# better62/MM-VQA-Healthcare

Hardware: AMD Instinct MI355X
Metric: image-question pairs/sec, M3AE-base fine-tune step (fwd+bwd+AdamW) @384px (higher is better)
Workload: dtype bf16

## Files before the change

### include/m3ae_hip.h

```cpp
#ifndef M3AE_HIP_H
#define M3AE_HIP_H

#include <stdint.h>

#ifdef __cplusplus
extern "C" {
#endif

#define M3AE_ABI_VERSION 4

enum { M3AE_F32 = 0, M3AE_BF16 = 1 };
enum { M3AE_ACT_NONE = 0, M3AE_ACT_GELU = 1, M3AE_ACT_QUICKGELU = 2, M3AE_ACT_TANH = 3, M3AE_ACT_RELU = 4,
       M3AE_ACT_MULAUX = 5  };
enum { M3AE_ERR_ARG = -1, M3AE_ERR_UNSUPPORTED = -2, M3AE_ERR_ALIGN = -3, M3AE_ERR_WORKSPACE = -4 };

int m3ae_abi_version(void);
void m3ae_desc_sizes(int64_t out3[3]);
const char* m3ae_last_gemm_path(void);

typedef struct {
    int64_t M, N, K;
    int64_t batch1, batch2;
    const void* A; int64_t a_sm, a_sk, a_sb1, a_sb2;
    const void* B; int64_t b_sk, b_sn, b_sb1, b_sb2;
    void* C;       int64_t c_sm, c_sn, c_sb1, c_sb2;
    int32_t dtype_a, dtype_b, dtype_c;
    float alpha;
    int32_t accumulate;
    const float* bias;
    int32_t act;
    void* preact;
    const void* residual;
    const void* dact_aux;
    int32_t dact;
    int32_t force_generic;
    float* a_rowsum;
    float dropout_p;
    uint64_t dropout_seed;
    int32_t preact_grad;
    int32_t launch_flags;
    const void* dropout_salt;
} m3ae_gemm_desc;
enum { M3AE_GEMM_NO_PERSISTENT = 1,
       M3AE_GEMM_F32_X3 = 2,
       M3AE_GEMM_DETERMINISTIC = 4,
       M3AE_GEMM_B_TILED = 8    };
#define M3AE_GEMM_NT_VARIANT(v) ((((v) + 1) & 0xf) << 8)
#define M3AE_GEMM_TN_VARIANT(v) ((((v) + 1) & 0xf) << 12)
#define M3AE_GEMM_COL_GROUP(g) (((g) & 0xf) << 16)
int m3ae_gemm(const m3ae_gemm_desc* d, void* stream);
int m3ae_gemm_rows(const m3ae_gemm_desc* d, int64_t row_base, int64_t row_step, void* stream);
int64_t m3ae_gemm_det_workspace_bytes(const m3ae_gemm_desc* d);
int m3ae_gemm_det(const m3ae_gemm_desc* d, void* workspace, int64_t workspace_bytes, void* stream);

typedef struct {
    int64_t B, H, Lq, Lk, Dh;
    const void* q; int64_t q_sb, q_sl;
    const void* k; int64_t k_sb, k_sl;
    const void* v; int64_t v_sb, v_sl;
    void* o;       int64_t o_sb, o_sl;
    const float* key_mask;
    const float* pos_bias;
    float scale;
    int32_t causal;
    float* lse; int64_t lse_stride;
    int32_t dtype;
    void* workspace; int64_t workspace_bytes;
    const void* d_o;
    void* dq; void* dk; void* dv;
    float* delta;
    float* d_pos_bias;
    float dropout_p;
    uint64_t dropout_seed;
    const void* dropout_salt;
    int32_t launch_flags;
} m3ae_attn_desc;
enum { M3AE_ATTN_LEGACY_KERNELS = 1,
       M3AE_ATTN_F32_X3 = 2    };
int64_t m3ae_attn_workspace_bytes(const m3ae_attn_desc* d, int backward);
int m3ae_attn_fwd(const m3ae_attn_desc* d, void* stream);
int m3ae_attn_bwd(const m3ae_attn_desc* d, void* stream);
int m3ae_attn_fwd_rows(const m3ae_attn_desc* d, int64_t row_base, int64_t row_step, void* stream);
int m3ae_attn_bwd_rows(const m3ae_attn_desc* d, int64_t row_base, int64_t row_step, void* stream);
int m3ae_attn_probs(const m3ae_attn_desc* d, float* probs, int64_t p_sb, int64_t p_sh, int64_t p_sq, void* stream);

typedef struct {
    int32_t dir;
    int64_t B, Lq, Lk, D, H;
    const void* x;
    const void* y;
    const float* key_mask;
    const void *wq, *wq_t, *wkv, *wkv_t, *wo, *wo_t;
    const float *bq, *bkv, *bo, *ln_g, *ln_b;
    float ln_eps;
    float dropout_p;
    uint64_t seed_attn, seed_hidden;
    void* proj;
    void* prime;
    float* colbias;
    void* probs;
    void* probs_drop;
    float* rowsum;
    void* zctx;
    void* ctx;
    void* s;
    void* out;
    float *mean, *rstd;
    const void* d_out;
    void* dx;
    void* dy;
    float *g_wq, *g_wkv, *g_wo, *g_bq, *g_bkv, *g_bo, *g_ln_g, *g_ln_b;
    void* ws_ds;
    void* ws_dsd;
    void* ws_dscores;
    void* ws_dprime;
    void* ws_dproj;
    void* ws_dz;
    void* ws_dctx;
    float* ws_vec;
    float* ws_ln;
    int32_t launch_flags;
    const void* dropout_salt;
} m3ae_xattn_desc;
enum { M3AE_XATTN_NO_PERSISTENT = 1,
       M3AE_XATTN_LEGACY_CHAIN = 2     };
int m3ae_xattn_supported(const m3ae_xattn_desc* d);
int m3ae_xattn_bwd_supported(const m3ae_xattn_desc* d);
int64_t m3ae_xattn_probs_ld(const m3ae_xattn_desc* d);
int m3ae_xattn_fwd(const m3ae_xattn_desc* d, void* stream);
int m3ae_xattn_bwd(const m3ae_xattn_desc* d, void* stream);
int m3ae_xattn_probs_export(const m3ae_xattn_desc* d, int dropped, float* out, int64_t o_sb, int64_t o_sh, int64_t o_sq,
                            void* stream);

int m3ae_layernorm_fwd(const void* x, const float* gamma, const float* beta, void* y, float* mean, float* rstd,
// ... 135 lines not shown
```

### mm-vqa-healthcare_amd/csrc/gemm_mfma.hip

```cpp
#include "gemm_nt_common.h"
#include "launch.h"
#include <stdlib.h>

namespace {

constexpr int BM = 128, BN = 128, BK = 64;
constexpr int STAGE_BYTES = (BM + BN) * BK * 2;
constexpr int LDS_BYTES = 2 * STAGE_BYTES;

using namespace m3g;

template <int BM_, int BN_, int BKT, int NST, int WM, int EPI>
__global__ __launch_bounds__((BM_ / WM) * (BN_ / 64) * 64, 2) void gemm_nt_bf16_kernel(MfmaArgs a) {
    if (a.has_drop) drop_resolve(a.drop);
    constexpr int WAVES_N = BN_ / 64, NWAVES = (BM_ / WM) * WAVES_N, MI = WM / 16;
    constexpr int A_BYTES = BM_ * BKT * 2, ST_BYTES = (BM_ + BN_) * BKT * 2;
    constexpr int A_SEGS = A_BYTES / 1024 / NWAVES, B_SEGS = BN_ * BKT * 2 / 1024 / NWAVES;
    constexpr int G = A_SEGS + B_SEGS;
    extern __shared__ __attribute__((aligned(16))) char smem[];
    const int tid = threadIdx.x;
    const int lane = tid & 63;
    const int wave = __builtin_amdgcn_readfirstlane(tid >> 6);
    const int wr = wave / WAVES_N, wc = wave % WAVES_N;

// ... 282 lines not shown
            for (int j = 0; j < 4; ++j)
                acc[i][j] = __builtin_amdgcn_mfma_f32_16x16x32_bf16(
                    __builtin_bit_cast(bf16x8_t, bfr[j]), __builtin_bit_cast(bf16x8_t, af[i]), acc[i][j], 0, 0, 0);
        __builtin_amdgcn_s_setprio(0);
        PP_FENCE();
        __builtin_amdgcn_s_barrier();
        PP_FENCE();
#pragma unroll
        for (int i = 0; i < 4; ++i) af[i] = nt_frag<CK>(At, wr * 128 + 64 + i * 16 + frow, fchunk);
        if (more) nt_stage<CK, 2, NW>(a.A, a.lda, m0, a.M, (int64_t)(c + 3) * CK, nxt, wave, lane);
        {
            const int rem = nc - 1 - c;
            if (rem >= 3) asm volatile("s_waitcnt vmcnt(8)" ::: "memory");
            else if (rem == 2) asm volatile("s_waitcnt vmcnt(4)" ::: "memory");
            else asm volatile("s_waitcnt vmcnt(0)" ::: "memory");
        }
        PP_FENCE();
        __builtin_amdgcn_s_barrier();
        PP_FENCE();
        asm volatile("s_waitcnt lgkmcnt(0)" ::: "memory");
        __builtin_amdgcn_sched_barrier(0);
        __builtin_amdgcn_s_setprio(1);
#pragma unroll
        for (int i = 0; i < 4; ++i)
#pragma unroll
            for (int j = 0; j < 4; ++j)
                acc[4 + i][j] = __builtin_amdgcn_mfma_f32_16x16x32_bf16(
                    __builtin_bit_cast(bf16x8_t, bfr[j]), __builtin_bit_cast(bf16x8_t, af[i]), acc[4 + i][j], 0, 0, 0);
        __builtin_amdgcn_s_setprio(0);
        PP_FENCE();
        __builtin_amdgcn_s_barrier();
        PP_FENCE();
    }
    if (wr == 0) { __builtin_amdgcn_s_barrier(); PP_FENCE(); }

    if (a.rows_epi) {
        if (a.c_f32) epilogue_rows<float, EPI, 8>(a, smem, wave, lane, m0 + wr * 128, n0 + wc * 64, acc);
        else epilogue_rows<bf16_t, EPI, 8>(a, smem, wave, lane, m0 + wr * 128, n0 + wc * 64, acc);
        return;
    }
#pragma unroll
    for (int i = 0; i < 8; ++i) {
        const int64_t m = m0 + wr * 128 + i * 16 + (lane & 15);
        if (m >= a.M) continue;
#pragma unroll
        for (int j = 0; j < 4; ++j) {
            const int64_t n = n0 + wc * 64 + j * 16 + 4 * (lane >> 4);
            if (n >= a.N) continue;
            if (a.c_f32) epilogue4<float, EPI>(a, m, n, acc[i][j]);
            else epilogue4<bf16_t, EPI>(a, m, n, acc[i][j]);
        }
    }
}

template <int EPI>
static int launch_nt_pp(const MfmaArgs& a, hipStream_t s) {
    constexpr int lds = 4 * (256 + 256) * 32 * 2;
    const int64_t tiles = cdiv(a.M, 256) * cdiv(a.N, 256);
    return launch_dyn<gemm_nt_pp_kernel<EPI>>(dim3((unsigned)tiles), dim3(512), lds, s, a);
}

enum NtKernel { NT_T128, NT_T256, NT_PP, NT_PP2, NT_PP2_PERSISTENT };

static NtKernel nt_kernel_choice(const MfmaArgs& a) {
    const bool both = a.M > 128 && a.N > 128;
    const bool pp2_ok = both && a.rows_epi && a.K >= 256;
    if (a.nt_variant >= 0) {
        switch (a.nt_variant) {
        case 9: return pp2_ok ? NT_PP2 : NT_T128;
        case 10: return pp2_ok ? NT_PP2_PERSISTENT : NT_T128;
        case 7: return both ? NT_PP : NT_T128;
        case 4: return both ? NT_T256 : NT_T128;
        default: return NT_T128;
        }
    }
    const int64_t t256 = cdiv(a.M, 256) * cdiv(a.N, 256), t128 = cdiv(a.M, 128) * cdiv(a.N, 128);
    const double eff256 = (double)t256 / (double)(cdiv(t256, 256) * 256);
    const double eff128 = (double)t128 / (double)(cdiv(t128, 512) * 512);
    if (!both || eff256 < 0.93 * eff128) return NT_T128;
    if (!pp2_ok) return NT_PP;
    return t256 >= 512 && !a.no_persist ? NT_PP2_PERSISTENT : NT_PP2;
}

template <int EPI>
static int launch_nt_v(const MfmaArgs& a, hipStream_t s) {
    const NtKernel k = nt_kernel_choice(a);
    g_last_path = k == NT_PP ? "mfma_nt_pp" : (k == NT_PP2 || k == NT_PP2_PERSISTENT) ? "mfma_nt_pp2" : "mfma_nt";
    switch (k) {
    case NT_PP2: return launch_nt_pp2(a, EPI, false, s);
    case NT_PP2_PERSISTENT: return launch_nt_pp2(a, EPI, true, s);
    case NT_PP: return launch_nt_pp<EPI>(a, s);
    case NT_T256: return launch_nt_t<256, 256, 64, 2, 128, EPI>(a, s);
    default: return launch_nt_t<128, 128, 64, 2, 64, EPI>(a, s);
    }
}


static int launch_nt(const m3ae_gemm_desc& d, hipStream_t s, DropRows rows) {
    MfmaArgs a{};
    a.A = (const bf16_t*)d.A; a.lda = d.a_sm;
    a.B = (const bf16_t*)d.B; a.ldb = d.b_sn;
    a.C = d.C; a.ldc = d.c_sm;
    a.M = d.M; a.N = d.N; a.K = d.K;
    a.c_f32 = d.dtype_c == M3AE_F32;
    a.alpha = d.alpha; a.accumulate = d.accumulate; a.bias = d.bias; a.act = d.act; a.preact = d.preact;
    a.preact_grad = d.preact_grad;
    a.residual = d.residual; a.dact_aux = d.dact_aux; a.dact = d.dact;
    a.rows_epi = (d.N % 8 == 0 && d.c_sm % 8 == 0) ? 1 : 0;
    {
        const int tiles_n = (int)((d.N + 255) / 256);
        const int g_nt_col_group = (d.launch_flags >> 16) & 0xf;
        a.col_group = g_nt_col_group > 0 ? g_nt_col_group : (tiles_n <= 9 ? tiles_n : 6);
    }
    a.has_drop = d.dropout_p > 0.f;
    a.drop = make_drop(d.dropout_p, d.dropout_seed, d.dropout_salt, rows);
    a.no_persist = (d.launch_flags & M3AE_GEMM_NO_PERSISTENT) ? 1 : 0;
    a.nt_variant = ((d.launch_flags >> 8) & 0xf) - 1;
    a.b_tiled = (d.launch_flags & M3AE_GEMM_B_TILED) ? 1 : 0;
    a.st_policy = (d.launch_flags >> 20) & 0x3;
    if (a.st_policy == 0) a.st_policy = (d.M * d.N >= (int64_t)16 << 20) ? 3 : 1;
    const bool has_act = d.act != M3AE_ACT_NONE, has_dact = d.dact_aux != nullptr;
    if (!has_act && !has_dact && !d.preact) return launch_nt_v<EPI_PLAIN>(a, s);
    if (!has_dact && d.act == M3AE_ACT_RELU) return launch_nt_v<EPI_RELU>(a, s);
    if (!has_act && has_dact && d.dact == M3AE_ACT_MULAUX) return launch_nt_v<EPI_DMUL>(a, s);
    if (a.has_drop) return launch_nt_v<EPI_ANY>(a, s);
    if (!has_dact && d.act == M3AE_ACT_GELU) return launch_nt_v<EPI_GELU>(a, s);
    if (!has_dact && d.act == M3AE_ACT_QUICKGELU) return launch_nt_v<EPI_QGELU>(a, s);
    if (!has_act && d.dact == M3AE_ACT_GELU) return launch_nt_v<EPI_DGELU>(a, s);
    if (!has_act && d.dact == M3AE_ACT_QUICKGELU) return launch_nt_v<EPI_DQGELU>(a, s);
    return launch_nt_v<EPI_ANY>(a, s);
}


#ifdef M3AE_TN_TRACE
__device__ uint64_t g_tn_trace[512 * 2 * 16];
#define TN_STAMP(k) do { if (tn_tr) g_tn_trace[((size_t)blockIdx.x * 2 + wr) * 16 + (k)] = __builtin_readcyclecounter(); } while (0)
extern "C" int m3ae_tn_trace_dump(uint64_t* out) {
    hipDeviceSynchronize();
    hipMemcpyFromSymbol(out, HIP_SYMBOL(g_tn_trace), sizeof(uint64_t) * 512 * 2 * 16);
    static uint64_t zeros[512 * 2 * 16];
    hipMemcpyToSymbol(HIP_SYMBOL(g_tn_trace), zeros, sizeof(zeros));
    return 0;
}
#else
#define TN_STAMP(k) do { } while (0)
#endif
template <bool DET>
__global__ __launch_bounds__(512, 2) void gemm_tn_pp_kernel(MfmaArgs a) {
    constexpr int CK = 32, NW = 8, A_BYTES = 256 * CK * 2, SLOT = 2 * A_BYTES;
    extern __shared__ __attribute__((aligned(16))) char smem[];
    const int tid = threadIdx.x;
    const int lane = tid & 63;
    const int wave = __builtin_amdgcn_readfirstlane(tid >> 6);
    const int wr = wave >> 2, wc = wave & 3;

    const unsigned tiles_n = (unsigned)(a.N / 256);
    const unsigned tiles = (unsigned)(a.M / 256) * tiles_n;
    const unsigned wg = xcd_remap(blockIdx.x, gridDim.x);
    const unsigned tile_id = wg % tiles, split = wg / tiles;
    const int64_t m0 = (int64_t)(tile_id / tiles_n) * 256;
    const int64_t n0 = (int64_t)(tile_id % tiles_n) * 256;
    const int64_t r_begin = (int64_t)split * a.k_chunk;
    int64_t r_end = r_begin + a.k_chunk;
    if (r_end > a.K) r_end = a.K;
    if (r_begin >= r_end) return;
    const int nc = (int)((r_end - r_begin + CK - 1) / CK);

    f32x4 acc[8][4];
#pragma unroll
    for (int i = 0; i < 8; ++i)
#pragma unroll
        for (int j = 0; j < 4; ++j) acc[i][j] = (f32x4){0.f, 0.f, 0.f, 0.f};
    const bool do_rowsum = a.a_rowsum != nullptr && n0 == 0 && wc == 0;
    f32x4 rsum[8];
#pragma unroll
    for (int i = 0; i < 8; ++i) rsum[i] = (f32x4){0.f, 0.f, 0.f, 0.f};
    const s16x8 ones = {0x3F80, 0x3F80, 0x3F80, 0x3F80, 0x3F80, 0x3F80, 0x3F80, 0x3F80};

#pragma unroll
    for (int c = 0; c < 3; ++c) {
        if (c < nc) {
            const int64_t r0 = r_begin + (int64_t)c * CK;
            tn_stage<256, 2, NW>(a.B, a.ldb, r0, r_end, n0, smem + c * SLOT + A_BYTES, wave, lane);
            tn_stage<256, 2, NW>(a.A, a.lda, r0, r_end, m0, smem + c * SLOT, wave, lane);
        }
    }
    if (nc >= 3) asm volatile("s_waitcnt vmcnt(8)" ::: "memory");
    else if (nc == 2) asm volatile("s_waitcnt vmcnt(4)" ::: "memory");
    else asm volatile("s_waitcnt vmcnt(0)" ::: "memory");
    PP_FENCE();
    __builtin_amdgcn_s_barrier();
    PP_FENCE();
    if (wr == 1) { __builtin_amdgcn_s_barrier(); PP_FENCE(); }

    for (int c = 0; c < nc; ++c) {
#ifdef M3AE_TN_TRACE
        const bool tn_tr = (c == 64 || c == 65) && lane == 0 && wc == 0 && blockIdx.x < 512;
        if (tn_tr && c == 65) g_tn_trace[((size_t)blockIdx.x * 2 + wr) * 16 + 8] = __builtin_readcyclecounter();
#undef TN_STAMP
#define TN_STAMP(k) do { if (tn_tr && c == 64) g_tn_trace[((size_t)blockIdx.x * 2 + wr) * 16 + (k)] = __builtin_readcyclecounter(); } while (0)
#endif
        TN_STAMP(0);
        const char* At = smem + (c & 3) * SLOT;
        const char* Bt = At + A_BYTES;
        char* nxt = smem + ((c + 3) & 3) * SLOT;
        const bool more = c + 3 < nc;
        const int64_t r3 = r_begin + (int64_t)(c + 3) * CK;
        s16x8 bfr[4], af[4];
#pragma unroll
        for (int j = 0; j < 4; ++j) bfr[j] = tn_frag<256>(Bt, 0, wc * 64 + j * 16, lane);
#pragma unroll
        for (int i = 0; i < 4; ++i) af[i] = tn_frag<256>(At, 0, wr * 128 + i * 16, lane);
        if (more) tn_stage<256, 2, NW>(a.B, a.ldb, r3, r_end, n0, nxt + A_BYTES, wave, lane);
// ... 212 lines not shown
}

static int tn_kernel_choice(const m3ae_gemm_desc& d) {
    const bool pp_ok = d.M % 256 == 0 && d.N % 256 == 0 && d.K >= 4096;
    const int g_tn_variant = ((d.launch_flags >> 12) & 0xf) - 1;
    if (g_tn_variant == 5 && pp_ok) return 5;
    if (g_tn_variant < 0 || g_tn_variant == 6) {
        const bool r3_rule = pp_ok && (d.K >= 65536 || (d.K >= 32768 && d.M * d.N >= 768 * 3072));
        const bool r4_rule = pp_ok && d.K >= 65536 && d.M * d.N >= 768 * 3072;
        if (g_tn_variant == 6 ? r3_rule : r4_rule) return 5;
        return 2;
    }
    if (g_tn_variant == 2) return 2;
    return 0;
}

static int launch_tn(const m3ae_gemm_desc& d, hipStream_t s, float* det_ws = nullptr) {
    MfmaArgs a{};
    a.A = (const bf16_t*)d.A; a.lda = d.a_sk;
    a.B = (const bf16_t*)d.B; a.ldb = d.b_sk;
    a.C = d.C; a.ldc = d.c_sm;
    a.M = d.M; a.N = d.N; a.K = d.K;
    a.c_f32 = 1; a.alpha = d.alpha; a.accumulate = d.accumulate; a.a_rowsum = d.a_rowsum;
    const int k = tn_kernel_choice(d);
    if (k == 5) return launch_tn_pp(a, d, s, det_ws);
    if (k == 2) return launch_tn_t<128, 128, 64, 32, 2>(a, d, s, det_ws);
    return launch_tn_t<128, 128, 64, 64, 2>(a, d, s, det_ws);
}


enum GemmRoute { ROUTE_BAD_DIMS, ROUTE_F32X3, ROUTE_NT, ROUTE_TN, ROUTE_GENERIC };
static GemmRoute gemm_route(const m3ae_gemm_desc& d) {
    if (d.M <= 0 || d.N <= 0 || d.K <= 0 || d.batch1 <= 0 || d.batch2 <= 0) return ROUTE_BAD_DIMS;
    if ((d.launch_flags & M3AE_GEMM_F32_X3) && !d.force_generic) return ROUTE_F32X3;
    const bool bf = d.dtype_a == M3AE_BF16 && d.dtype_b == M3AE_BF16;
    const bool single = d.batch1 == 1 && d.batch2 == 1;
    if (bf && single && !d.force_generic && d.c_sn == 1) {
        const bool ptr_ok = aligned16(d.A) && aligned16(d.B) && aligned16(d.C) &&
                            (!d.preact || aligned16(d.preact)) && (!d.residual || aligned16(d.residual)) &&
                            (!d.dact_aux || aligned16(d.dact_aux)) && (!d.bias || aligned16(d.bias));
        if (ptr_ok && !d.a_rowsum && d.a_sk == 1 && d.b_sk == 1 && d.K % BK == 0 && d.N % 4 == 0 && d.a_sm % 8 == 0 &&
            d.b_sn % 8 == 0 && d.c_sm % 4 == 0)
            return ROUTE_NT;
        if (ptr_ok && d.a_sm == 1 && d.b_sn == 1 && d.dtype_c == M3AE_F32 && d.M % BM == 0 && d.N % BN == 0 &&
            d.a_sk % 8 == 0 && d.b_sk % 8 == 0 && !d.bias && d.act == M3AE_ACT_NONE && !d.preact && !d.residual &&
            !d.dact_aux)
            return ROUTE_TN;
    }
    return ROUTE_GENERIC;
}

extern "C" int m3ae_gemm(const m3ae_gemm_desc* dp, void* stream) { return m3ae_gemm_rows(dp, 0, 1, stream); }

extern "C" int m3ae_gemm_rows(const m3ae_gemm_desc* dp, int64_t row_base, int64_t row_step, void* stream) {
    if (!dp || !dp->A || !dp->B || !dp->C) return M3AE_ERR_ARG;
    const m3ae_gemm_desc& d = *dp;
    const GemmRoute route = gemm_route(d);
    if (route == ROUTE_BAD_DIMS) return M3AE_ERR_ARG;
    const DropRows rows{row_base, row_step};
    if (!drop_rows_ok(rows, d.M, d.N)) return M3AE_ERR_ARG;
    if ((d.launch_flags & M3AE_GEMM_B_TILED) &&
        (d.dtype_a != M3AE_BF16 || d.dtype_b != M3AE_BF16 || d.b_sk != 1 || d.b_sn != d.K || d.K % 32 != 0 || d.batch1 != 1 ||
         d.batch2 != 1 || (d.launch_flags & M3AE_GEMM_F32_X3) || !aligned16(d.B)))
        return M3AE_ERR_UNSUPPORTED;
    if (route == ROUTE_TN && d.dropout_p > 0.f && (row_base != 0 || row_step != 1)) return M3AE_ERR_UNSUPPORTED;
    if (d.launch_flags & M3AE_GEMM_DETERMINISTIC) return M3AE_ERR_UNSUPPORTED;
    hipStream_t s = (hipStream_t)stream;
    switch (route) {
    case ROUTE_F32X3:
        if (d.dtype_a != M3AE_F32 || d.dtype_b != M3AE_F32 || d.dtype_c != M3AE_F32) return M3AE_ERR_UNSUPPORTED;
        g_last_path = "f32x3";
        return m3ae_gemm_f32x3(d, s, rows);
    case ROUTE_NT:
        return launch_nt(d, s, rows);
    case ROUTE_TN:
        g_last_path = "mfma_tn";
        return launch_tn(d, s);
    default:
        g_last_path = "generic";
        return m3ae_gemm_generic(d, s, rows);
    }
}

extern "C" int64_t m3ae_gemm_det_workspace_bytes(const m3ae_gemm_desc* dp) {
    if (!dp) return M3AE_ERR_ARG;
    const m3ae_gemm_desc& d = *dp;
    if (gemm_route(d) != ROUTE_TN) return 0;
    int64_t k_chunk = 0;
    const int k = tn_kernel_choice(d);
    const int64_t splits = k == 5 ? tn_pp_splits(d, &k_chunk) : tn_t_splits(d, tn_t_lds(2, k == 2 ? 32 : 64), &k_chunk);
    return tn_det_bytes(d, splits);
}

extern "C" int m3ae_gemm_det(const m3ae_gemm_desc* dp, void* workspace, int64_t workspace_bytes, void* stream) {
    if (!dp || !dp->A || !dp->B || !dp->C) return M3AE_ERR_ARG;
    const m3ae_gemm_desc& d = *dp;
    if (!(d.launch_flags & M3AE_GEMM_DETERMINISTIC)) return M3AE_ERR_ARG;
    if (d.launch_flags & M3AE_GEMM_B_TILED) return M3AE_ERR_UNSUPPORTED;
    if (gemm_route(d) != ROUTE_TN) return M3AE_ERR_UNSUPPORTED;
    if (!workspace || !aligned16(workspace) || workspace_bytes < m3ae_gemm_det_workspace_bytes(dp)) return M3AE_ERR_WORKSPACE;
    g_last_path = "mfma_tn";
    return launch_tn(d, (hipStream_t)stream, (float*)workspace);
}
```

### mm-vqa-healthcare_amd/m3ae_amd/_lib.py

```python
import ctypes as C
import os

_PKG = os.path.dirname(os.path.abspath(__file__))
DIAGNOSTIC = os.environ.get("M3AE_DIAGNOSTIC_LIB", "") == "1"
LIB_PATH = os.path.join(_PKG, "lib_diag" if DIAGNOSTIC else "lib", "libm3ae_hip.so")

F32, BF16 = 0, 1
ACT_NONE, ACT_GELU, ACT_QUICKGELU, ACT_TANH, ACT_RELU, ACT_MULAUX = 0, 1, 2, 3, 4, 5

vp, i64, i32, f32 = C.c_void_p, C.c_int64, C.c_int32, C.c_float


class GemmDesc(C.Structure):
    _fields_ = [
        ("M", i64), ("N", i64), ("K", i64), ("batch1", i64), ("batch2", i64),
        ("A", vp), ("a_sm", i64), ("a_sk", i64), ("a_sb1", i64), ("a_sb2", i64),
        ("B", vp), ("b_sk", i64), ("b_sn", i64), ("b_sb1", i64), ("b_sb2", i64),
        ("C", vp), ("c_sm", i64), ("c_sn", i64), ("c_sb1", i64), ("c_sb2", i64),
        ("dtype_a", i32), ("dtype_b", i32), ("dtype_c", i32),
        ("alpha", f32), ("accumulate", i32), ("bias", vp), ("act", i32), ("preact", vp), ("residual", vp),
        ("dact_aux", vp), ("dact", i32), ("force_generic", i32), ("a_rowsum", vp),
        ("dropout_p", f32), ("dropout_seed", C.c_uint64), ("preact_grad", i32), ("launch_flags", i32), ("dropout_salt", vp),
    ]


class AttnDesc(C.Structure):
    _fields_ = [
        ("B", i64), ("H", i64), ("Lq", i64), ("Lk", i64), ("Dh", i64),
        ("q", vp), ("q_sb", i64), ("q_sl", i64),
        ("k", vp), ("k_sb", i64), ("k_sl", i64),
        ("v", vp), ("v_sb", i64), ("v_sl", i64),
        ("o", vp), ("o_sb", i64), ("o_sl", i64),
        ("key_mask", vp), ("pos_bias", vp), ("scale", f32), ("causal", i32),
        ("lse", vp), ("lse_stride", i64), ("dtype", i32), ("workspace", vp), ("workspace_bytes", i64),
        ("d_o", vp), ("dq", vp), ("dk", vp), ("dv", vp), ("delta", vp), ("d_pos_bias", vp),
        ("dropout_p", f32), ("dropout_seed", C.c_uint64), ("dropout_salt", vp), ("launch_flags", i32),
    ]


class XattnDesc(C.Structure):
    _fields_ = [
        ("dir", i32), ("B", i64), ("Lq", i64), ("Lk", i64), ("D", i64), ("H", i64),
        ("x", vp), ("y", vp), ("key_mask", vp),
        ("wq", vp), ("wq_t", vp), ("wkv", vp), ("wkv_t", vp), ("wo", vp), ("wo_t", vp),
        ("bq", vp), ("bkv", vp), ("bo", vp), ("ln_g", vp), ("ln_b", vp),
        ("ln_eps", f32), ("dropout_p", f32), ("seed_attn", C.c_uint64), ("seed_hidden", C.c_uint64),
        ("proj", vp), ("prime", vp), ("colbias", vp), ("probs", vp), ("probs_drop", vp), ("rowsum", vp),
        ("zctx", vp), ("ctx", vp), ("s", vp), ("out", vp), ("mean", vp), ("rstd", vp),
        ("d_out", vp), ("dx", vp), ("dy", vp),
        ("g_wq", vp), ("g_wkv", vp), ("g_wo", vp), ("g_bq", vp), ("g_bkv", vp), ("g_bo", vp), ("g_ln_g", vp), ("g_ln_b", vp),
        ("ws_ds", vp), ("ws_dsd", vp), ("ws_dscores", vp), ("ws_dprime", vp), ("ws_dproj", vp), ("ws_dz", vp), ("ws_dctx", vp),
        ("ws_vec", vp), ("ws_ln", vp), ("launch_flags", i32), ("dropout_salt", vp),
    ]


GEMM_NO_PERSISTENT, GEMM_F32_X3, GEMM_DETERMINISTIC, GEMM_B_TILED = 1, 2, 4, 8
DET_COLSUM, DET_EMBED_BWD, DET_BCE, DET_XENT, DET_MIM = 0, 1, 2, 3, 4
ATTN_LEGACY_KERNELS, ATTN_F32_X3 = 1, 2
XATTN_NO_PERSISTENT, XATTN_LEGACY_CHAIN = 1, 2
CLIP_NORM, CLIP_COEF, CLIP_SKIP, CLIP_STEPS, CLIP_CLIPPED_STEPS, CLIP_SKIPPED_STEPS, CLIP_RECORD_WORDS = 0, 1, 2, 4, 5, 6, 8
ABI_VERSION = 4


_SIGS = {
    "m3ae_abi_version": (C.c_int, []),
    "m3ae_desc_sizes": (None, [C.POINTER(i64)]),
    "m3ae_last_gemm_path": (C.c_char_p, []),
    "m3ae_gemm": (C.c_int, [C.POINTER(GemmDesc), vp]),
    "m3ae_attn_workspace_bytes": (i64, [C.POINTER(AttnDesc), C.c_int]),
    "m3ae_attn_fwd": (C.c_int, [C.POINTER(AttnDesc), vp]),
    "m3ae_attn_bwd": (C.c_int, [C.POINTER(AttnDesc), vp]),
    "m3ae_attn_probs": (C.c_int, [C.POINTER(AttnDesc), vp, i64, i64, i64, vp]),
    "m3ae_xattn_supported": (C.c_int, [C.POINTER(XattnDesc)]),
    "m3ae_xattn_bwd_supported": (C.c_int, [C.POINTER(XattnDesc)]),
    "m3ae_xattn_probs_ld": (i64, [C.POINTER(XattnDesc)]),
    "m3ae_xattn_fwd": (C.c_int, [C.POINTER(XattnDesc), vp]),
    "m3ae_xattn_bwd": (C.c_int, [C.POINTER(XattnDesc), vp]),
    "m3ae_xattn_probs_export": (C.c_int, [C.POINTER(XattnDesc), C.c_int, vp, i64, i64, i64, vp]),
    "m3ae_layernorm_fwd": (C.c_int, [vp, vp, vp, vp, vp, vp, i64, i64, f32, C.c_int, C.c_int, C.c_int, vp]),
    "m3ae_layernorm_bwd_blocks": (i64, [i64]),
    "m3ae_layernorm_bwd": (C.c_int, [vp, vp, vp, vp, vp, vp, vp, vp, vp, vp, vp, i64, i64, C.c_int, C.c_int, C.c_int, vp]),
    "m3ae_layernorm_bwd_drop": (C.c_int, [vp, vp, vp, vp, vp, vp, vp, vp, f32, C.c_uint64, vp, vp, vp, vp, i64, i64, C.c_int, vp]),
    "m3ae_dropout": (C.c_int, [vp, vp, vp, i64, i64, f32, C.c_uint64, vp, C.c_int, vp]),
    "m3ae_colsum": (C.c_int, [vp, vp, i64, i64, i64, C.c_int, C.c_int, vp]),
    "m3ae_roberta_embed_fwd": (C.c_int, [vp, vp, vp, vp, vp, i64, i64, i64, i64, C.c_int, vp]),
    "m3ae_roberta_embed_bwd": (C.c_int, [vp, vp, vp, vp, vp, i64, i64, i64, i64, C.c_int, vp]),
    "m3ae_patchify": (C.c_int, [vp, vp, i64, i64, i64, C.c_int, vp]),
    "m3ae_image_normalize_u8": (C.c_int, [vp, vp, i64, i64, i64, C.POINTER(C.c_float), C.POINTER(C.c_float), vp]),
    "m3ae_vit_tokens_fwd": (C.c_int, [vp, vp, vp, vp, i64, i64, i64, C.c_int, vp]),
    "m3ae_vit_tokens_bwd": (C.c_int, [vp, vp, vp, vp, i64, i64, i64, C.c_int, vp]),
    "m3ae_bce_logits": (C.c_int, [vp, vp, vp, vp, i64, i64, f32, C.c_int, vp]),
    "m3ae_xent": (C.c_int, [vp, vp, vp, vp, vp, i64, i64, i64, f32, C.c_int, vp]),
    "m3ae_adamw": (C.c_int, [vp, vp, vp, vp, vp, i64, f32, f32, f32, f32, f32, i64, f32, vp, vp]),
    "m3ae_cast_transpose": (C.c_int, [vp, vp, vp, i64, i64, vp]),
    "m3ae_cast_transpose_batched": (C.c_int, [vp, C.c_int, i64, vp]),
    "m3ae_transpose_bf16_batched": (C.c_int, [vp, C.c_int, i64, vp]),
    "m3ae_tile_bf16_batched": (C.c_int, [vp, C.c_int, i64, vp]),
    "m3ae_cast": (C.c_int, [vp, vp, i64, C.c_int, C.c_int, vp]),
    "m3ae_zero": (C.c_int, [vp, i64, vp]),
    "m3ae_add": (C.c_int, [vp, vp, vp, i64, C.c_int, vp]),
    "m3ae_act_fwd": (C.c_int, [vp, vp, i64, C.c_int, C.c_int, vp]),
    "m3ae_act_bwd": (C.c_int, [vp, vp, vp, i64, C.c_int, C.c_int, vp]),
    "m3ae_gather_rows": (C.c_int, [vp, vp, vp, i64, i64, C.c_int, vp]),
    "m3ae_scatter_add_rows": (C.c_int, [vp, vp, vp, i64, i64, C.c_int, vp]),
    "m3ae_mask_ranks": (C.c_int, [vp, vp, vp, vp, i64, i64, i64, vp]),
    "m3ae_mim_targets": (C.c_int, [vp, vp, i64, i64, i64, i64, i64, C.c_int, vp]),
    "m3ae_mim_loss_fwd": (C.c_int, [vp, vp, vp, vp, vp, i64, i64, i64, C.c_int, vp]),
    "m3ae_mim_loss_bwd": (C.c_int, [vp, vp, vp, vp, vp, vp, i64, i64, i64, C.c_int, vp]),
    "m3ae_selftest": (C.c_int, [vp, vp]),
    "m3ae_gemm_det_workspace_bytes": (i64, [C.POINTER(GemmDesc)]),
    "m3ae_gemm_det": (C.c_int, [C.POINTER(GemmDesc), vp, i64, vp]),
    "m3ae_det_workspace_bytes": (i64, [C.c_int, i64, i64]),
    "m3ae_colsum_det": (C.c_int, [vp, vp, i64, i64, i64, C.c_int, C.c_int, vp, i64, vp]),
    "m3ae_layernorm_bwd_det": (C.c_int, [vp, vp, vp, vp, vp, vp, vp, vp, vp, vp, vp, i64, i64, C.c_int, C.c_int, C.c_int, vp]),
    "m3ae_layernorm_bwd_drop_det": (C.c_int, [vp, vp, vp, vp, vp, vp, vp, vp, f32, C.c_uint64, vp, vp, vp, vp, i64, i64, C.c_int, vp]),
    "m3ae_roberta_embed_bwd_det": (C.c_int, [vp, vp, vp, vp, vp, i64, i64, i64, i64, C.c_int, vp, i64, vp]),
    "m3ae_bce_logits_det": (C.c_int, [vp, vp, vp, vp, i64, i64, f32, C.c_int, vp, i64, vp]),
    "m3ae_xent_det": (C.c_int, [vp, vp, vp, vp, i64, i64, i64, f32, C.c_int, vp, i64, vp]),
    "m3ae_mim_loss_fwd_det": (C.c_int, [vp, vp, vp, vp, vp, i64, i64, i64, C.c_int, vp, i64, vp]),
    "m3ae_image_resample_workspace_bytes": (i64, [i64, i64]),
    "m3ae_image_resample_u8": (C.c_int, [vp, i64, vp, vp, i64, i64, i64, vp, i64, vp, vp, C.POINTER(C.c_float), C.POINTER(C.c_float), vp]),
    "m3ae_image_resample_tables": (C.c_int, [vp, i64, i64, vp, i64, vp]),
    "m3ae_image_randaug_workspace_bytes": (i64, [i64]),
    "m3ae_image_randaug_u8": (C.c_int, [vp, vp, i64, vp, i64, vp, i64, C.c_int, vp]),
    "m3ae_gemm_rows": (C.c_int, [C.POINTER(GemmDesc), i64, i64, vp]),
    "m3ae_attn_fwd_rows": (C.c_int, [C.POINTER(AttnDesc), i64, i64, vp]),
    "m3ae_attn_bwd_rows": (C.c_int, [C.POINTER(AttnDesc), i64, i64, vp]),
    "m3ae_layernorm_bwd_drop_rows": (C.c_int, [vp, vp, vp, vp, vp, vp, vp, vp, f32, C.c_uint64, vp, vp, vp, vp, i64, i64, C.c_int, i64, i64, vp]),
    "m3ae_dropout_rows": (C.c_int, [vp, vp, vp, i64, i64, f32, C.c_uint64, vp, C.c_int, i64, i64, vp]),
    "m3ae_beam_topk_workspace_bytes": (i64, [i64, i64, i64, i64]),
    "m3ae_beam_topk": (C.c_int, [vp, i64, vp, i64, i64, i64, i64, vp, i64, vp, vp, vp]),
    "m3ae_beam_step": (C.c_int, [vp, vp, vp, vp, vp, vp, vp, vp, vp, vp, vp, vp, vp, vp, i64, i64, i64, i64, i64, i64, i64, C.c_double, vp]),
    "m3ae_beam_finalize": (C.c_int, [vp, vp, vp, vp, vp, vp, vp, vp, vp, i64, i64, i64, i64, i64, i64, C.c_double, vp]),
    "m3ae_expand_samples": (C.c_int, [vp, vp, vp, i64, i64, i64, C.c_int, vp]),
    "m3ae_segment_sum_rows": (C.c_int, [vp, vp, vp, vp, i64, i64, i64, C.c_int, vp]),
    "m3ae_sumsq_workspace_bytes": (i64, [i64]),
    "m3ae_sumsq_segments": (C.c_int, [vp, i64, vp, i64, vp, i64, vp, vp, i64, vp]),
    "m3ae_clip_finalize": (C.c_int, [vp, i64, f32, f32, vp, vp]),
    "m3ae_adamw_clip": (C.c_int, [vp, vp, vp, vp, vp, i64, f32, f32, f32, f32, f32, i64, f32, vp, vp, vp]),
    "m3ae_layernorm_fwd_mixed": (C.c_int, [vp, vp, vp, vp, vp, vp, i64, i64, f32, vp]),
    "m3ae_layernorm_bwd_mixed": (C.c_int, [vp, vp, vp, vp, vp, vp, vp, vp, vp, vp, vp, i64, i64, vp]),
    "m3ae_layernorm_bwd_mixed_det": (C.c_int, [vp, vp, vp, vp, vp, vp, vp, vp, vp, vp, vp, i64, i64, vp]),
}

EXPORTS = tuple(_SIGS)
_lib = None


class M3AEHipError(RuntimeError):
    pass


def lib():
    global _lib
    if _lib is None:
        if not os.path.exists(LIB_PATH):
            raise M3AEHipError(f"{LIB_PATH} is missing: build it with `python -m m3ae_amd.build` "
                               f"(or __graft_entry__.build()); this package has no CPU fallback")
        import torch
        if DIAGNOSTIC:
            import warnings
            warnings.warn(f"m3ae_amd: loading the DIAGNOSTIC library {LIB_PATH} (timing-only builds may compute wrong results)")
        l = C.CDLL(LIB_PATH)
        for name, (res, args) in _SIGS.items():
            fn = getattr(l, name)
            fn.restype, fn.argtypes = res, args
        if l.m3ae_abi_version() != ABI_VERSION:
            raise M3AEHipError(f"ABI version mismatch: library {l.m3ae_abi_version()}, binding {ABI_VERSION}")
        sizes = (i64 * 3)()
        l.m3ae_desc_sizes(sizes)
        mine = (C.sizeof(GemmDesc), C.sizeof(AttnDesc), C.sizeof(XattnDesc))
        if tuple(sizes) != mine:
            raise M3AEHipError(f"descriptor layout mismatch: library {tuple(sizes)}, binding {mine}")
        _lib = l
    return _lib


def check(rc, what):
    if rc != 0:
        kind = {-1: "invalid argument", -2: "unsupported shape/dtype", -3: "misaligned", -4: "workspace too small"}.get(
            rc, f"hipError_t {rc}" if rc > 0 else f"error {rc}")
        raise M3AEHipError(f"{what} failed: {kind}")
```

### mm-vqa-healthcare_amd/m3ae_amd/ops.py

```python
import contextlib
import ctypes as C
import functools
import math
import os
import threading
from typing import NamedTuple

import torch

from . import _lib
from ._lib import (ACT_GELU, ACT_MULAUX, ACT_NONE, ACT_QUICKGELU, ACT_RELU, ACT_TANH, BF16, F32, AttnDesc, GemmDesc, XattnDesc,
                   check)

grad_ready_hook = None
SAVE_DACT = os.environ.get("M3AE_SAVE_DACT", "1") != "0"
NT_NO_PERSISTENT = os.environ.get("M3AE_NT_NO_PERSISTENT", "0") == "1"
GEMM_NT_VARIANT, GEMM_TN_VARIANT, GEMM_COL_GROUP = int(os.environ.get("M3AE_GEMM_NT_VARIANT", -1)), int(os.environ.get("M3AE_GEMM_TN_VARIANT", -1)), int(os.environ.get("M3AE_GEMM_COL_GROUP", 0))


ATTN_LEGACY = os.environ.get("M3AE_ATTN_LEGACY", "0") == "1"
GEMM_ST_POLICY = int(os.environ.get("M3AE_GEMM_ST_POLICY", 0))
TILED_B = os.environ.get("M3AE_TILED_B", "1") != "0"


def _gemm_flags():
    return ((1 if NT_NO_PERSISTENT else 0) | (((GEMM_NT_VARIANT + 1) & 0xF) << 8) | (((GEMM_TN_VARIANT + 1) & 0xF) << 12)
            | ((GEMM_COL_GROUP & 0xF) << 16) | ((GEMM_ST_POLICY & 0x3) << 20))
PROFILE = None


class _Mode(threading.local):
    x3 = False


_MODE = _Mode()


@contextlib.contextmanager
def f32x3_mode(on):
    prev, _MODE.x3 = _MODE.x3, bool(on)
    try:
        yield
    finally:
        _MODE.x3 = prev


def f32x3_active():
    return _MODE.x3


def model_mode(fn):
    @functools.wraps(fn)
    def run(self, *args, **kwargs):
        with f32x3_mode(getattr(self, "f32x3", False)):
            return fn(self, *args, **kwargs)
    return run


class DeterministicError(_lib.M3AEHipError):
    pass


_DETERMINISTIC = False


def set_deterministic(on):
    global _DETERMINISTIC
    _DETERMINISTIC = bool(on)


def deterministic():
    return _DETERMINISTIC


@contextlib.contextmanager
def deterministic_mode(on=True):
    prev = deterministic()
    set_deterministic(on)
    try:
        yield
    finally:
        set_deterministic(prev)


def _no_ordered_form(op):
    if _DETERMINISTIC:
        raise DeterministicError(f"{op} has no deterministic form (it adds with fp32 atomics) and ops.deterministic() is on: "
                                 f"switch the mode off for this op with ops.set_deterministic(False)")


def _det_ws(nbytes, device):
    return torch.empty(max(int(nbytes), 16), dtype=torch.uint8, device=device)


def _small_ws(op, rows, cols, device):
    n = _lib.lib().m3ae_det_workspace_bytes(op, rows, cols)
    if n < 0:
        check(int(n), "m3ae_det_workspace_bytes")
    return _det_ws(n, device), n


class Function(torch.autograd.Function):

    def __init_subclass__(cls, **kwargs):
        super().__init_subclass__(**kwargs)
        fwd, bwd = cls.__dict__.get("forward"), cls.__dict__.get("backward")
        if fwd is not None:
            f = fwd.__func__ if isinstance(fwd, staticmethod) else fwd

            def forward(ctx, *args):
# ... 1666 lines not shown
```

Before: 1436.

## Split NT GEMMs into 256-tile head and 128-tile tail launches to cut wave quantization

For NT GEMMs where the default choice would be the 128x128 tile kernel, the launcher now splits M into a head covering whole rounds of 256x256 tiles and a tail of leftover rows. The head runs on the ping-pong PP2 kernel (persistent when large enough) and the tail runs through the normal kernel choice, with pointers for A, C, residual, preact, dact_aux and dropout rows offset to match. The aim is to get the bigger-tile efficiency on most of the matrix while avoiding the partially filled last wave of 256 tiles. The cost is an extra kernel launch, a tail kernel that may underfill the GPU, and a new flag plus query entry point to turn the split off.

```diff
diff --git a/include/m3ae_hip.h b/include/m3ae_hip.h
--- a/include/m3ae_hip.h
+++ b/include/m3ae_hip.h
@@ -48,8 +48,10 @@
 #define M3AE_GEMM_NT_VARIANT(v) ((((v) + 1) & 0xf) << 8)
 #define M3AE_GEMM_TN_VARIANT(v) ((((v) + 1) & 0xf) << 12)
 #define M3AE_GEMM_COL_GROUP(g) (((g) & 0xf) << 16)
+#define M3AE_GEMM_NT_NO_SPLIT (1 << 22)
 int m3ae_gemm(const m3ae_gemm_desc* d, void* stream);
 int m3ae_gemm_rows(const m3ae_gemm_desc* d, int64_t row_base, int64_t row_step, void* stream);
+int64_t m3ae_gemm_nt_split_rows(const m3ae_gemm_desc* d);
 int64_t m3ae_gemm_det_workspace_bytes(const m3ae_gemm_desc* d);
 int m3ae_gemm_det(const m3ae_gemm_desc* d, void* workspace, int64_t workspace_bytes, void* stream);
 
diff --git a/mm-vqa-healthcare_amd/csrc/gemm_mfma.hip b/mm-vqa-healthcare_amd/csrc/gemm_mfma.hip
--- a/mm-vqa-healthcare_amd/csrc/gemm_mfma.hip
+++ b/mm-vqa-healthcare_amd/csrc/gemm_mfma.hip
@@ -388,10 +388,31 @@
     return t256 >= 512 && !a.no_persist ? NT_PP2_PERSISTENT : NT_PP2;
 }
 
+#ifndef NT_SPLIT_TAIL_MAX
+#define NT_SPLIT_TAIL_MAX 0.9
+#endif
+#ifndef NT_SPLIT_MIN_ROUNDS_T128
+#define NT_SPLIT_MIN_ROUNDS_T128 3
+#endif
+static int64_t nt_split_rows(const MfmaArgs& a) {
+    if (a.nt_variant >= 0) return 0;
+    const NtKernel whole = nt_kernel_choice(a);
+    bool pp2 = false;
+#ifdef NT_SPLIT_FROM_PP2
+    pp2 = whole == NT_PP2 || whole == NT_PP2_PERSISTENT;
+#endif
+    const bool head_ok = a.M > 128 && a.N > 128 && a.rows_epi && a.K >= 256;
+    if (!pp2 && !(whole == NT_T128 && head_ok)) return 0;
+    const int64_t tiles_n = cdiv(a.N, 256), t256 = cdiv(a.M, 256) * tiles_n, full_rounds = t256 / 256;
+    if (full_rounds == 0 || t256 % 256 == 0 || (!pp2 && full_rounds < NT_SPLIT_MIN_ROUNDS_T128)) return 0;
+    const int64_t head = full_rounds * 256 / tiles_n * 256;
+    if (head <= 0) return 0;
+    const int64_t tail_rounds128 = cdiv(cdiv(a.M - head, 128) * cdiv(a.N, 128), 512);
+    return (double)tail_rounds128 * (0.5 / 0.93) <= NT_SPLIT_TAIL_MAX ? head : 0;
+}
+
 template <int EPI>
-static int launch_nt_v(const MfmaArgs& a, hipStream_t s) {
-    const NtKernel k = nt_kernel_choice(a);
-    g_last_path = k == NT_PP ? "mfma_nt_pp" : (k == NT_PP2 || k == NT_PP2_PERSISTENT) ? "mfma_nt_pp2" : "mfma_nt";
+static int launch_nt_k(const MfmaArgs& a, NtKernel k, hipStream_t s) {
     switch (k) {
     case NT_PP2: return launch_nt_pp2(a, EPI, false, s);
     case NT_PP2_PERSISTENT: return launch_nt_pp2(a, EPI, true, s);
@@ -399,6 +420,34 @@
     case NT_T256: return launch_nt_t<256, 256, 64, 2, 128, EPI>(a, s);
     default: return launch_nt_t<128, 128, 64, 2, 64, EPI>(a, s);
     }
+}
+
+template <int EPI>
+static int launch_nt_v(const MfmaArgs& a, hipStream_t s, bool no_split) {
+    const int64_t head_rows = no_split ? 0 : nt_split_rows(a);
+    if (head_rows > 0) {
+        MfmaArgs h = a, t = a;
+        h.M = head_rows;
+        const int64_t t256 = cdiv(h.M, 256) * cdiv(h.N, 256);
+        g_last_path = "mfma_nt_pp2";
+        const int rc = launch_nt_k<EPI>(h, t256 >= 512 && !a.no_persist ? NT_PP2_PERSISTENT : NT_PP2, s);
+        if (rc != 0) return rc;
+        const size_t csz = a.c_f32 ? 4 : 2;
+        t.M = a.M - head_rows;
+        t.A = a.A + head_rows * a.lda;
+        t.C = (char*)a.C + head_rows * a.ldc * csz;
+        if (a.residual) t.residual = (const char*)a.residual + head_rows * a.ldc * csz;
+        if (a.preact) t.preact = (char*)a.preact + head_rows * a.ldc * csz;
+        if (a.dact_aux) t.dact_aux = (const char*)a.dact_aux + head_rows * a.ldc * csz;
+        t.drop.row_base += head_rows * t.drop.row_step;
+#ifdef NT_SPLIT_TAIL_T128
+        return launch_nt_k<EPI>(t, NT_T128, s);
+#endif
+        return launch_nt_k<EPI>(t, nt_kernel_choice(t), s);
+    }
+    const NtKernel k = nt_kernel_choice(a);
+    g_last_path = k == NT_PP ? "mfma_nt_pp" : (k == NT_PP2 || k == NT_PP2_PERSISTENT) ? "mfma_nt_pp2" : "mfma_nt";
+    return launch_nt_k<EPI>(a, k, s);
 }
 
 
@@ -425,16 +474,17 @@
     a.b_tiled = (d.launch_flags & M3AE_GEMM_B_TILED) ? 1 : 0;
     a.st_policy = (d.launch_flags >> 20) & 0x3;
     if (a.st_policy == 0) a.st_policy = (d.M * d.N >= (int64_t)16 << 20) ? 3 : 1;
+    const bool no_split = (d.launch_flags & M3AE_GEMM_NT_NO_SPLIT) != 0;
     const bool has_act = d.act != M3AE_ACT_NONE, has_dact = d.dact_aux != nullptr;
-    if (!has_act && !has_dact && !d.preact) return launch_nt_v<EPI_PLAIN>(a, s);
-    if (!has_dact && d.act == M3AE_ACT_RELU) return launch_nt_v<EPI_RELU>(a, s);
-    if (!has_act && has_dact && d.dact == M3AE_ACT_MULAUX) return launch_nt_v<EPI_DMUL>(a, s);
-    if (a.has_drop) return launch_nt_v<EPI_ANY>(a, s);
-    if (!has_dact && d.act == M3AE_ACT_GELU) return launch_nt_v<EPI_GELU>(a, s);
-    if (!has_dact && d.act == M3AE_ACT_QUICKGELU) return launch_nt_v<EPI_QGELU>(a, s);
-    if (!has_act && d.dact == M3AE_ACT_GELU) return launch_nt_v<EPI_DGELU>(a, s);
-    if (!has_act && d.dact == M3AE_ACT_QUICKGELU) return launch_nt_v<EPI_DQGELU>(a, s);
-    return launch_nt_v<EPI_ANY>(a, s);
+    if (!has_act && !has_dact && !d.preact) return launch_nt_v<EPI_PLAIN>(a, s, no_split);
+    if (!has_dact && d.act == M3AE_ACT_RELU) return launch_nt_v<EPI_RELU>(a, s, no_split);
+    if (!has_act && has_dact && d.dact == M3AE_ACT_MULAUX) return launch_nt_v<EPI_DMUL>(a, s, no_split);
+    if (a.has_drop) return launch_nt_v<EPI_ANY>(a, s, no_split);
+    if (!has_dact && d.act == M3AE_ACT_GELU) return launch_nt_v<EPI_GELU>(a, s, no_split);
+    if (!has_dact && d.act == M3AE_ACT_QUICKGELU) return launch_nt_v<EPI_QGELU>(a, s, no_split);
+    if (!has_act && d.dact == M3AE_ACT_GELU) return launch_nt_v<EPI_DGELU>(a, s, no_split);
+    if (!has_act && d.dact == M3AE_ACT_QUICKGELU) return launch_nt_v<EPI_DQGELU>(a, s, no_split);
+    return launch_nt_v<EPI_ANY>(a, s, no_split);
 }
 
 
@@ -813,6 +863,18 @@
     }
 }
 
+extern "C" int64_t m3ae_gemm_nt_split_rows(const m3ae_gemm_desc* dp) {
+    if (!dp) return M3AE_ERR_ARG;
+    const m3ae_gemm_desc& d = *dp;
+    if (gemm_route(d) != ROUTE_NT || (d.launch_flags & M3AE_GEMM_NT_NO_SPLIT)) return 0;
+    MfmaArgs a{};
+    a.M = d.M; a.N = d.N; a.K = d.K;
+    a.rows_epi = (d.N % 8 == 0 && d.c_sm % 8 == 0) ? 1 : 0;
+    a.no_persist = (d.launch_flags & M3AE_GEMM_NO_PERSISTENT) ? 1 : 0;
+    a.nt_variant = ((d.launch_flags >> 8) & 0xf) - 1;
+    return nt_split_rows(a);
+}
+
 extern "C" int64_t m3ae_gemm_det_workspace_bytes(const m3ae_gemm_desc* dp) {
     if (!dp) return M3AE_ERR_ARG;
     const m3ae_gemm_desc& d = *dp;
diff --git a/mm-vqa-healthcare_amd/m3ae_amd/_lib.py b/mm-vqa-healthcare_amd/m3ae_amd/_lib.py
--- a/mm-vqa-healthcare_amd/m3ae_amd/_lib.py
+++ b/mm-vqa-healthcare_amd/m3ae_amd/_lib.py
@@ -55,6 +55,7 @@
 
 
 GEMM_NO_PERSISTENT, GEMM_F32_X3, GEMM_DETERMINISTIC, GEMM_B_TILED = 1, 2, 4, 8
+GEMM_NT_NO_SPLIT = 1 << 22
 DET_COLSUM, DET_EMBED_BWD, DET_BCE, DET_XENT, DET_MIM = 0, 1, 2, 3, 4
 ATTN_LEGACY_KERNELS, ATTN_F32_X3 = 1, 2
 XATTN_NO_PERSISTENT, XATTN_LEGACY_CHAIN = 1, 2
@@ -124,6 +125,7 @@
     "m3ae_image_randaug_workspace_bytes": (i64, [i64]),
     "m3ae_image_randaug_u8": (C.c_int, [vp, vp, i64, vp, i64, vp, i64, C.c_int, vp]),
     "m3ae_gemm_rows": (C.c_int, [C.POINTER(GemmDesc), i64, i64, vp]),
+    "m3ae_gemm_nt_split_rows": (i64, [C.POINTER(GemmDesc)]),
     "m3ae_attn_fwd_rows": (C.c_int, [C.POINTER(AttnDesc), i64, i64, vp]),
     "m3ae_attn_bwd_rows": (C.c_int, [C.POINTER(AttnDesc), i64, i64, vp]),
     "m3ae_layernorm_bwd_drop_rows": (C.c_int, [vp, vp, vp, vp, vp, vp, vp, vp, f32, C.c_uint64, vp, vp, vp, vp, i64, i64, C.c_int, i64, i64, vp]),
diff --git a/mm-vqa-healthcare_amd/m3ae_amd/ops.py b/mm-vqa-healthcare_amd/m3ae_amd/ops.py
--- a/mm-vqa-healthcare_amd/m3ae_amd/ops.py
+++ b/mm-vqa-healthcare_amd/m3ae_amd/ops.py
@@ -20,12 +20,13 @@
 
 ATTN_LEGACY = os.environ.get("M3AE_ATTN_LEGACY", "0") == "1"
 GEMM_ST_POLICY = int(os.environ.get("M3AE_GEMM_ST_POLICY", 0))
+GEMM_NT_NO_SPLIT = os.environ.get("M3AE_GEMM_NT_NO_SPLIT", "0") == "1"
 TILED_B = os.environ.get("M3AE_TILED_B", "1") != "0"
 
 
 def _gemm_flags():
     return ((1 if NT_NO_PERSISTENT else 0) | (((GEMM_NT_VARIANT + 1) & 0xF) << 8) | (((GEMM_TN_VARIANT + 1) & 0xF) << 12)
-            | ((GEMM_COL_GROUP & 0xF) << 16) | ((GEMM_ST_POLICY & 0x3) << 20))
+            | ((GEMM_COL_GROUP & 0xF) << 16) | ((GEMM_ST_POLICY & 0x3) << 20) | (_lib.GEMM_NT_NO_SPLIT if GEMM_NT_NO_SPLIT else 0))
 PROFILE = None
 
 
```

Result: no change. 1430 (-0.4%).
